# nanless/universal-speech-enhancement

Hardware: AMD Instinct MI355X
Metric: spectrogram-frames/sec through 30-step PC sampler, 24 kHz (higher is better)
Workload: dtype bf16; 1 GPU; configs[1]: NCSN++ Large score net, batch=8x4 s utterances per GPU, 30-step PC sampler (reverse_diffusion + langevin x1, snr 0.5, 60 NFE), bf16, hipGraph=on; global_batch=8, frames_per_utt=601, padded_frames_per_utt=640, n_freq=512, N=30, nfe=60, parallelism=utterance-sharded x1

## Files before the change

universal_speech_enhancement_amd/csrc/use_conv_sk.hip:

```cpp
#include "use_kernels.h"
#include <type_traits>
#include "use_device.h"

namespace use {

namespace {

template <typename T> struct SkMma;
template <> struct SkMma<__bf16> {
    DEVI static f32x16 mma(const uint4 a, const uint4 b, f32x16 c) {
        return __builtin_amdgcn_mfma_f32_32x32x16_bf16(__builtin_bit_cast(bf16x8, a), __builtin_bit_cast(bf16x8, b), c, 0, 0, 0);
    }
};
template <> struct SkMma<_Float16> {
    DEVI static f32x16 mma(const uint4 a, const uint4 b, f32x16 c) {
        return __builtin_amdgcn_mfma_f32_32x32x16_f16(__builtin_bit_cast(f16x8, a), __builtin_bit_cast(f16x8, b), c, 0, 0, 0);
    }
};
template <> struct SkMma<float> {
    DEVI static f32x16 mma(const uint4 a, const uint4 b, f32x16 c) {
        const float4 fa = __builtin_bit_cast(float4, a), fb = __builtin_bit_cast(float4, b);
        c = __builtin_amdgcn_mfma_f32_32x32x2f32(fa.x, fb.x, c, 0, 0, 0);
        c = __builtin_amdgcn_mfma_f32_32x32x2f32(fa.y, fb.y, c, 0, 0, 0);
        c = __builtin_amdgcn_mfma_f32_32x32x2f32(fa.z, fb.z, c, 0, 0, 0);
        c = __builtin_amdgcn_mfma_f32_32x32x2f32(fa.w, fb.w, c, 0, 0, 0);
        return c;
    }
};

constexpr int SK_HPMAX = 128;
constexpr int SK_MT = 64;

template <typename TIN, typename TOUT, int NJ, int CP>
__global__ __launch_bounds__(512) void conv_sk_kernel(ConvArgs p, int TH, int TW) {
    constexpr int ES = (int)sizeof(TIN);
    constexpr int VEC = 16 / ES;
    constexpr int NP = ES;
    constexpr int MI = SK_MT / 32, MT = SK_MT, NT = 32 * NJ;
    constexpr int ROWB = CP * ES + 16;
    constexpr int UMAX = (9 * (CP / 32) + 7) / 8;
    constexpr int NPC = SK_HPMAX * (CP * ES / 16) / 512;
    constexpr int NTP = NT + 8;
    constexpr int HALO_BYTES = SK_HPMAX * ROWB, RED_BYTES = 4 * MT * NTP * 4;
    constexpr int SMEM = HALO_BYTES > RED_BYTES ? HALO_BYTES : RED_BYTES;
    constexpr bool ACC = ES == 4;
    static_assert(NPC >= 1 && SK_HPMAX * (CP * ES / 16) % 512 == 0, "halo staging");
    __shared__ __attribute__((aligned(16))) char smem[SMEM];
    __shared__ float2 coef_s[1024];
    __shared__ float2 st_red[8][NT];

    const int tid = threadIdx.x, lane = tid & 63, wave = tid >> 6;
    const int b = blockIdx.z, n0 = blockIdx.y * NT;
    const int pad = p.ntaps == 9 ? 1 : 0;
    const int tiles_x = (p.W + TW - 1) / TW;
    const int ty0 = (blockIdx.x / tiles_x) * TH, tx0 = (blockIdx.x % tiles_x) * TW;
    const int HW_ = TW + 2 * pad, HP = HW_ * (TH + 2 * pad);
    const int Ctot = p.C0 + p.C1, XCtot = p.XC0 + p.XC1;
    const bool has_gn = p.coef || p.gn_st0;

    f32x16 acc[MI][NJ];
#pragma unroll
    for (int i = 0; i < MI; ++i)
#pragma unroll
        for (int j = 0; j < NJ; ++j)
#pragma unroll
            for (int r = 0; r < 16; ++r) acc[i][j][r] = 0.f;

    int a_off[MI];
#pragma unroll
    for (int i = 0; i < MI; ++i) {
        int m = i * 32 + (lane & 31);
        if (m >= TH * TW) m = 0;
        const int ty = m / TW;
        a_off[i] = (ty * HW_ + (m - ty * TW)) * ROWB + (lane >> 5) * 16;
    }

    bool first = true;
    for (int si = 0; si < 4; ++si) {
        const bool seg1 = si >= 2;
        const TIN* src = (const TIN*)(si == 0 ? p.src0 : si == 1 ? p.src1 : si == 2 ? p.x0 : p.x1);
        const int Cs = si == 0 ? p.C0 : si == 1 ? p.C1 : si == 2 ? p.XC0 : p.XC1;
        const int cg0 = si == 1 ? p.C0 : si == 3 ? p.XC0 : 0;
        const char* wbase = seg1 ? (const char*)p.w2 : (const char*)p.w;
        const int wld = seg1 ? XCtot : Ctot, wtaps = seg1 ? 1 : p.ntaps;
        const bool use_coef = has_gn && !seg1, use_act = p.act && !seg1;
        const char* wslab = seg1 ? (const char*)p.w2b : (const char*)p.wb;
        constexpr int SCK = ES == 4 ? 16 : 32;
        const int nslabs = wld / SCK;
        for (int c_loc = 0; c_loc < Cs; c_loc += CP) {
            const int pc = Cs - c_loc < CP ? Cs - c_loc : CP;
            const int cpu_ = pc >> 5;
            const int nunits = wtaps * cpu_;
            const int c_glob = cg0 + c_loc;
            const int d_tap = 8 / cpu_, d_chunk = 8 - d_tap * cpu_;
            const int tap0 = wave / cpu_, chunk0 = wave - tap0 * cpu_;
            uint4 bw[UMAX][NJ][NP];
            {
                int tap = tap0, chunk = chunk0;
#pragma unroll
                for (int i = 0; i < UMAX; ++i) {
                    if (wave + 8 * i < nunits) {
#pragma unroll
                        for (int j = 0; j < NJ; ++j) {
                            int row = n0 + j * 32 + (lane & 31);
#ifdef USE_HIP_ABLATE
                            if (p.dbg & 1) row = n0 + j * 32 + (lane & 1);
#endif
                            if (wslab) {
#pragma unroll
                                for (int q = 0; q < NP; ++q) {
                                    const int cgl = c_glob + chunk * 32 + (2 * q + (lane >> 5)) * VEC;
                                    const int slab = cgl / SCK, piece = (cgl % SCK) / VEC;
                                    bw[i][j][q] = *reinterpret_cast<const uint4*>(
                                        wslab + (((size_t)tap * nslabs + slab) * p.cout_pad + row) * 64 + ((piece ^ ((row >> 2) & 3)) << 4));
                                }
                            } else {
                                const char* wp = wbase + (((size_t)row * wtaps + tap) * wld + c_glob + chunk * 32) * ES + (lane >> 5) * 16;
#pragma unroll
                                for (int q = 0; q < NP; ++q) bw[i][j][q] = *reinterpret_cast<const uint4*>(wp + q * 32);
                            }
                        }
                    }
                    tap += d_tap; chunk += d_chunk;
                    if (chunk >= cpu_) { chunk -= cpu_; ++tap; }
                }
            }
            if (first) {
                if (has_gn) gn_fill_table(coef_s, p, b, Ctot, tid, 512);
                first = false;
            }
            __syncthreads();
            const int ppp = pc * ES / 16;
            const int npieces = HP * ppp;
            const int d_pix = 512 / ppp, d_part = 512 - d_pix * ppp;
            const int d_hy = d_pix / HW_, d_hx = d_pix - d_hy * HW_;
            uint4 raw[NPC];
            int loff[NPC];
            {
                int pix = tid / ppp, part = tid - pix * ppp;
                int hy = pix / HW_, hx = pix - hy * HW_;
#pragma unroll
                for (int k = 0; k < NPC; ++k) {
                    raw[k] = make_uint4(0, 0, 0, 0);
                    loff[k] = 0;
                    if (tid + k * 512 < npieces) {
                        const int gy = ty0 + hy - pad, gx = tx0 + hx - pad;
                        const bool inb = gy >= 0 && gy < p.H && gx >= 0 && gx < p.W;
                        loff[k] = (pix * ROWB + part * 16) | (inb ? 0x40000000 : 0) | 0x80000000;
                        if (inb) raw[k] = *reinterpret_cast<const uint4*>(src + ((size_t)(b * p.H + gy) * p.W + gx) * Cs + c_loc + part * VEC);
                    }
                    part += d_part; pix += d_pix; hx += d_hx; hy += d_hy;
                    if (part >= ppp) { part -= ppp; ++pix; ++hx; }
                    if (hx >= HW_) { hx -= HW_; ++hy; }
                }
            }
            {
                int part = tid % ppp;
#pragma unroll
                for (int k = 0; k < NPC; ++k) {
                    if (loff[k] < 0) {
                        uint4 o = raw[k];
#ifdef USE_HIP_ABLATE
                        if (p.dbg & 2) { *reinterpret_cast<uint4*>(smem + (loff[k] & 0x3fffffff)) = o; continue; }
#endif
                        if ((loff[k] & 0x40000000) && (use_coef || use_act)) {
                            float v[VEC];
                            Vec16<TIN>::load(reinterpret_cast<const TIN*>(&o), v);
                            if (use_coef) {
                                const float2* cf = coef_s + c_glob + part * VEC;
#pragma unroll
                                for (int e = 0; e < VEC; ++e) { const float2 ab = cf[e]; v[e] = fmaf(v[e], ab.x, ab.y); }
                            }
                            if (use_act) {
#pragma unroll
                                for (int e = 0; e < VEC; ++e) v[e] = silu_f<ACC>(v[e]);
                            }
                            o = Vec16<TIN>::pack(v);
                        }
                        *reinterpret_cast<uint4*>(smem + (loff[k] & 0x3fffffff)) = o;
                    }
                    part += d_part;
                    if (part >= ppp) part -= ppp;
                }
            }
            __syncthreads();
            {
                int tap = tap0, chunk = chunk0;
#pragma unroll
                for (int i = 0; i < UMAX; ++i) {
#ifdef USE_HIP_ABLATE
                    if (p.dbg & 4) { if (wave + 8 * i < nunits) { _Pragma("unroll") for (int j = 0; j < NJ; ++j) _Pragma("unroll") for (int q = 0; q < NP; ++q) acc[0][j][q] += __builtin_bit_cast(float, bw[i][j][q].x); } continue; }
#endif
                    if (wave + 8 * i < nunits) {
                        const int dy = seg1 ? pad : (pad ? (tap * 11) >> 5 : 0);
                        const int dx = seg1 ? pad : (pad ? tap - dy * 3 : 0);
                        const char* ha = smem + (dy * HW_ + dx) * ROWB + chunk * 32 * ES;
#pragma unroll
                        for (int q = 0; q < NP; ++q) {
                            uint4 af[MI];
#pragma unroll
                            for (int m = 0; m < MI; ++m) af[m] = *reinterpret_cast<const uint4*>(ha + a_off[m] + q * 32);
#pragma unroll
                            for (int m = 0; m < MI; ++m)
#pragma unroll
                                for (int j = 0; j < NJ; ++j) acc[m][j] = SkMma<TIN>::mma(af[m], bw[i][j][q], acc[m][j]);
                        }
                    }
                    tap += d_tap; chunk += d_chunk;
                    if (chunk >= cpu_) { chunk -= cpu_; ++tap; }
                }
            }
        }
    }

    float* const red = reinterpret_cast<float*>(smem);
    float* const mine = red + (wave & 3) * (MT * NTP);
    __syncthreads();
#define SK_FOR_ACC(BODY)                                                                                   \
    _Pragma("unroll") for (int m = 0; m < MI; ++m) _Pragma("unroll") for (int j = 0; j < NJ; ++j)          \
    _Pragma("unroll") for (int r = 0; r < 16; ++r) {                                                       \
        const int row = m * 32 + (r & 3) + 8 * (r >> 2) + 4 * (lane >> 5), col = j * 32 + (lane & 31);     \
        BODY;                                                                                              \
    }
    if (wave >= 4) { SK_FOR_ACC(mine[row * NTP + col] = acc[m][j][r]) }
    __syncthreads();
    if (wave < 4) { SK_FOR_ACC(mine[row * NTP + col] += acc[m][j][r]) }
    __syncthreads();
#undef SK_FOR_ACC

    constexpr int CH = 16 / (int)sizeof(TOUT);
    constexpr int CPR = NT / CH;
    constexpr int ITEMS = MT * CPR;
    static_assert(512 % CPR == 0 && (CPR == 4 || CPR == 8 || CPR == 16), "epilogue chunking");
    TOUT* out = (TOUT*)p.out;
    const TOUT* res = (const TOUT*)p.res;
    const int ch = tid % CPR;
    const int co0 = n0 + ch * CH;
    float addv[CH], st_s[CH], st_q[CH];
    const int nvalid = p.Cout - co0;
#pragma unroll
    for (int c = 0; c < CH; ++c) {
        float add = 0.f;
        if (c < nvalid) {
            if (p.bias) add += p.bias[co0 + c];
            if (p.temb) add += p.temb[(size_t)b * p.temb_bstride + co0 + c];
        }
        addv[c] = add; st_s[c] = 0.f; st_q[c] = 0.f;
    }
#pragma unroll
    for (int it0 = 0; it0 < ITEMS; it0 += 512) {
        const int it = it0 + tid;
        const int row = it / CPR;
        if (it < ITEMS && row < TH * TW && nvalid > 0) {
            const int ty = row / TW, gy = ty0 + ty, gx = tx0 + row - ty * TW;
            if (gy < p.H && gx < p.W) {
                float v[CH];
#pragma unroll
                for (int c = 0; c < CH; ++c) v[c] = addv[c];
#pragma unroll
                for (int w = 0; w < 4; ++w)
#pragma unroll
                    for (int c4 = 0; c4 < CH / 4; ++c4) {
                        const float4 t4 = *reinterpret_cast<const float4*>(red + w * (MT * NTP) + row * NTP + ch * CH + c4 * 4);
                        v[c4 * 4] += t4.x; v[c4 * 4 + 1] += t4.y; v[c4 * 4 + 2] += t4.z; v[c4 * 4 + 3] += t4.w;
                    }
                const size_t pix = (size_t)(b * p.H + gy) * p.W + gx;
                if (res) {
                    float rv[CH];
                    if (nvalid >= CH) Vec16<TOUT>::load(res + pix * p.Cout + co0, rv);
                    else {
#pragma unroll
                        for (int c = 0; c < CH; ++c) rv[c] = c < nvalid ? to_f(res[pix * p.Cout + co0 + c]) : 0.f;
                    }
#pragma unroll
                    for (int c = 0; c < CH; ++c) v[c] += rv[c];
                }
#pragma unroll
                for (int c = 0; c < CH; ++c) v[c] *= p.out_scale;
                if (p.pyr && nvalid >= CH) {
                    const float4 pq = *reinterpret_cast<const float4*>(p.pyr + pix * 4);
#pragma unroll
                    for (int c = 0; c < CH; ++c) {
                        const float4 wq = *reinterpret_cast<const float4*>(p.w4 + (size_t)(co0 + c) * 4);
                        v[c] += p.b4[co0 + c] + wq.x * pq.x + wq.y * pq.y + wq.z * pq.z + wq.w * pq.w;
                    }
                }
                const uint4 packed = Vec16<TOUT>::pack(v);
                if (nvalid >= CH) *reinterpret_cast<uint4*>(out + pix * p.Cout + co0) = packed;
                else {
#pragma unroll
                    for (int c = 0; c < CH; ++c) if (c < nvalid) out[pix * p.Cout + co0 + c] = reinterpret_cast<const TOUT*>(&packed)[c];
                }
                float vr[CH];
                Vec16<TOUT>::load(reinterpret_cast<const TOUT*>(&packed), vr);
#pragma unroll
                for (int c = 0; c < CH; ++c) { st_s[c] += vr[c]; st_q[c] += vr[c] * vr[c]; }
            }
        }
    }
    if (p.stats) {
        constexpr int NWV = ITEMS / 64 < 8 ? ITEMS / 64 : 8;
#pragma unroll
        for (int c = 0; c < CH; ++c) { st_s[c] = reduce_lanes_stride<CPR>(st_s[c]); st_q[c] = reduce_lanes_stride<CPR>(st_q[c]); }
        if (lane < CPR && wave < NWV) {
#pragma unroll
            for (int c = 0; c < CH; ++c) st_red[wave][ch * CH + c] = make_float2(st_s[c], st_q[c]);
        }
        __syncthreads();
        if (tid < NT) {
            float ss = 0.f, qq = 0.f;
#pragma unroll
            for (int w = 0; w < NWV; ++w) { const float2 t = st_red[w][tid]; ss += t.x; qq += t.y; }
            if (n0 + tid < p.Cout) gn_accumulate(p.stats + ((size_t)b * p.Cout + n0 + tid) * 2, ss, qq);
        }
    }
}

long g_sk_max_px = 16L * 20L;

void sk_tile(int H, int W, int pad, int* th, int* tw) {
    long best = -1; int bh = 1, bw = 1;
    for (int w = 1; w <= W && w <= SK_MT; ++w) {
        int hmax = SK_MT / w; if (hmax > H) hmax = H;
        const int ny = (H + hmax - 1) / hmax;
        const int h = (H + ny - 1) / ny;
        const int halo = (h + 2 * pad) * (w + 2 * pad);
        if (halo > SK_HPMAX) continue;
        const long tiles = (long)ny * ((W + w - 1) / w);
        const long key = tiles * 1024 + halo;
        if (best < 0 || key < best) { best = key; bh = h; bw = w; }
    }
    *th = bh; *tw = bw;
}

template <typename T, typename TO, int NJ, int CP>
void sk_launch(const ConvArgs& a, int th, int tw, hipStream_t s) {
    const int tiles = ((a.H + th - 1) / th) * ((a.W + tw - 1) / tw);
    hipLaunchKernelGGL((conv_sk_kernel<T, TO, NJ, CP>), dim3(tiles, (a.Cout + 32 * NJ - 1) / (32 * NJ), a.B), dim3(512), 0, s, a, th, tw);
}

}

void conv_sk_set_max_px(long n) { g_sk_max_px = n; }

bool conv_sk_eligible(const ConvArgs& a) {
    const int Ctot = a.C0 + a.C1, XC = a.XC0 + a.XC1;
    const bool full = a.in_dtype == a.out_dtype && a.Cout % 32 == 0 && a.Cout >= 32;
    const bool head = a.out_dtype == DT_F32 && a.Cout <= 8 && a.cout_pad >= 32 && !a.pyr && !a.stats;
    const long max_px = (a.in_dtype == DT_F32 && g_sk_max_px > 0) ? std::max(g_sk_max_px, 4096L) : g_sk_max_px;
    return (long)a.H * a.W <= max_px && (a.ntaps == 9 || a.ntaps == 1) && a.w && (full || head) &&
           Ctot % 32 == 0 && a.C0 % 32 == 0 && XC % 32 == 0 && a.XC0 % 32 == 0 && (XC == 0 || a.w2) && Ctot >= 32 && Ctot <= 1024;
}

void launch_conv_sk(const ConvArgs& a, hipStream_t s) {
    int th, tw;
    sk_tile(a.H, a.W, a.ntaps == 9 ? 1 : 0, &th, &tw);
    const long tiles = (long)((a.H + th - 1) / th) * ((a.W + tw - 1) / tw) * a.B;
    const bool wide = a.Cout % 64 == 0 && tiles * (a.Cout / 32) > 512;
    if (a.in_dtype != a.out_dtype) {
        if (a.in_dtype == DT_BF16) sk_launch<__bf16, float, 1, 256>(a, th, tw, s); else sk_launch<_Float16, float, 1, 256>(a, th, tw, s);
        return;
    }
    if (a.in_dtype == DT_BF16)     { wide ? sk_launch<__bf16, __bf16, 2, 128>(a, th, tw, s) : sk_launch<__bf16, __bf16, 1, 256>(a, th, tw, s); }
    else if (a.in_dtype == DT_F16) { wide ? sk_launch<_Float16, _Float16, 2, 128>(a, th, tw, s) : sk_launch<_Float16, _Float16, 1, 256>(a, th, tw, s); }
    else                           { wide ? sk_launch<float, float, 2, 64>(a, th, tw, s) : sk_launch<float, float, 1, 128>(a, th, tw, s); }
}

}
```

universal_speech_enhancement_amd/csrc/use_engine.cpp:

```cpp
#include "../../include/use_hip.h"
#include "use_kernels.h"

#include <hip/hip_runtime.h>

#include <algorithm>
#include <cmath>
#include <cstdarg>
#include <cstdio>
#include <cstdlib>
#include <cstring>
#include <map>
#include <mutex>
#include <string>
#include <unordered_map>
#include <vector>

using namespace use;

static thread_local std::string g_err;
static int fail(int code, const char* fmt, ...) {
    char buf[1024];
    va_list ap; va_start(ap, fmt); vsnprintf(buf, sizeof buf, fmt, ap); va_end(ap);
    g_err = buf;
    return code;
// ... 810 lines not shown
}

static int ensure_sde_scratch(use_handle* h) {
    if (!h) return fail(USE_E_INVALID, "null handle");
    HIPCHK(hipSetDevice(h->device));
    if (!h->sde_buf) {
        const size_t bytes = 512 + (size_t)use_handle::SDE_MAX_B * use_handle::SDE_BLOCKS * 2 * 4;
        HIPCHK(hipMalloc((void**)&h->sde_buf, bytes));
        HIPCHK(hipMemset(h->sde_buf, 0, bytes));
        h->sde_rng = (unsigned long long*)h->sde_buf; h->sde_step = (float*)(h->sde_buf + 256);
        h->sde_partial = (float*)(h->sde_buf + 512);
    }
    return USE_OK;
}

static int ensure_cap_stream(use_handle* h) {
    if (!h->cap_stream) HIPCHK(hipStreamCreateWithFlags(&h->cap_stream, hipStreamNonBlocking));
    return USE_OK;
}

extern "C" {

int use_get_stat(use_handle* h, const char* name, long long* value) {
    if (!h || !name || !value) return fail(USE_E_INVALID, "null argument");
    if (!strcmp(name, "graph_captures")) { *value = h->n_graph_captures; return USE_OK; }
    if (!strcmp(name, "plans_built")) { *value = h->n_plans_built; return USE_OK; }
    if (!strcmp(name, "plan_cache_hits")) { *value = h->n_plan_cache_hits; return USE_OK; }
    if (!strcmp(name, "plans_parked")) { *value = (long long)h->plan_cache.size(); return USE_OK; }
    if (!strcmp(name, "ode_steps")) { *value = h->ode_steps; return USE_OK; }
    if (!strcmp(name, "ode_rejected")) { *value = h->ode_rejected; return USE_OK; }
    if (!strcmp(name, "ode_nfev_max")) { *value = h->ode_nfev_max; return USE_OK; }
    if (!strcmp(name, "plan_stale")) { *value = h->B && h->opt_gen_at_plan != g_opt_gen ? 1 : 0; return USE_OK; }
    return fail(USE_E_INVALID, "unknown statistic '%s'", name);
}

int use_set_option(const char* name, long long value) {
    if (!name) return fail(USE_E_INVALID, "option name is null");
    ++g_opt_gen;
    if (!strcmp(name, "attn_fused")) { g_attn_fused = (int)value; return USE_OK; }
    if (!strcmp(name, "plan_cache")) { g_plan_cache = (int)std::max(0LL, std::min(16LL, value)); return USE_OK; }
    if (!strcmp(name, "subbatch_min_items")) { g_subbatch_min_items = (int)std::max(1LL, value); return USE_OK; }
    if (!strcmp(name, "subbatch")) { g_subbatch = (int)value; return USE_OK; }
    if (!strcmp(name, "stagger_level")) { g_stagger_level = (int)value; return USE_OK; }
    if (!strcmp(name, "stats_part")) { g_stats_part = (int)value; return USE_OK; }
    if (!strcmp(name, "gn_inline")) { g_gn_inline = (long)value; return USE_OK; }
    if (!strcmp(name, "conv_v4_min_blocks")) { conv_v4_set_min_blocks((long)value); return USE_OK; }
    if (!strcmp(name, "conv_v5")) { conv_v5_set((int)value); return USE_OK; }
    if (!strcmp(name, "fir_strip")) { fir_set_strip((int)value); return USE_OK; }
    if (!strcmp(name, "pyr_ws")) { pyr_conv_set_ws((int)value); return USE_OK; }
    if (!strcmp(name, "wgrad_mfma16")) { wgrad_set_mfma16((int)value); return USE_OK; }
    if (!strcmp(name, "wgrad_blocks")) { wgrad_set_blocks((int)value); return USE_OK; }
    if (!strcmp(name, "conv_in_wgs")) { if (value < 1 || value > 4096) return fail(USE_E_INVALID, "conv_in_wgs: 1 ... 4096"); g_conv_in_wgs = (int)value; return USE_OK; }
    if (!strcmp(name, "conv_sk_max_px")) { conv_sk_set_max_px((long)value); return USE_OK; }
    return fail(USE_E_INVALID, "unknown option '%s'", name);
}
const char* use_last_error(void) { return g_err.c_str(); }
const char* use_version(void) { return "use_hip 0.1 (gfx950)"; }

int use_create(const use_config* cfg, int device, use_handle** out) {
    if (!cfg || !out) return fail(USE_E_INVALID, "null argument");
    if (cfg->n_levels < 1 || cfg->n_levels > 8 || cfg->nf % 32 != 0 || cfg->nf < 32 || cfg->num_res_blocks < 1)
        return fail(USE_E_INVALID, "unsupported architecture (nf must be a multiple of 32, 1..8 levels)");
    for (int i = 0; i < cfg->n_levels; ++i)
        if (cfg->ch_mult[i] < 1 || cfg->nf * cfg->ch_mult[i] > 512) return fail(USE_E_INVALID, "unsupported architecture (1 <= nf * ch_mult <= 512)");
    if (cfg->n_freq % (1 << (cfg->n_levels - 1)) != 0)
        return fail(USE_E_INVALID, "n_freq=%d is not divisible by 2^(levels-1)", cfg->n_freq);
    if (cfg->precision != USE_PREC_FP32 && cfg->precision != USE_PREC_BF16 && cfg->precision != USE_PREC_FP16) return fail(USE_E_INVALID, "bad precision");
    if (cfg->input_channels != 0 && cfg->input_channels != 2 && cfg->input_channels != 4 && cfg->input_channels != 6)
        return fail(USE_E_INVALID, "input_channels must be 4 (x and y), 6 (x, y and a second conditioning) or 2 (y alone), got %d", cfg->input_channels);
    use_handle* h = new use_handle();
    h->cfg = *cfg; h->device = device;
    h->act_dtype = cfg->precision == USE_PREC_BF16 ? DT_BF16 : cfg->precision == USE_PREC_FP16 ? DT_F16 : DT_F32;
    int rc = build_arch(h);
    if (rc) { delete h; return rc; }
    *out = h;
    return USE_OK;
}

int use_destroy(use_handle* h) {
    if (!h) return USE_OK;
    (void)hipSetDevice(h->device);
    (void)hipDeviceSynchronize();
    drop_graphs(h); plan_cache_clear(h);
    if (h->ode_run) (void)use_ode_destroy(h->ode_run);
    if (h->cap_stream) (void)hipStreamDestroy(h->cap_stream);
    for (int i = 0; i < MAX_SUB; ++i) {
        if (h->aux_stream[i]) (void)hipStreamDestroy(h->aux_stream[i]);
        if (h->ev_stagger[i]) { (void)hipEventDestroy(h->ev_stagger[i]); (void)hipEventDestroy(h->ev_join[i]); }
    }
    if (h->ev_fork) (void)hipEventDestroy(h->ev_fork);
    if (h->blob) (void)hipFree(h->blob);
    if (h->arena.base) (void)hipFree(h->arena.base);
    if (h->persist) (void)hipFree(h->persist);
    if (h->temb_table) (void)hipFree(h->temb_table);
    if (h->silu_table) (void)hipFree(h->silu_table);
    if (h->ts_dev) (void)hipFree(h->ts_dev);
    if (h->noise_copy) (void)hipFree(h->noise_copy);
    if (h->sde_buf) (void)hipFree(h->sde_buf);
    delete h;
    return USE_OK;
}

int use_num_expected_weights(use_handle* h) { return h ? (int)h->expected.size() : USE_E_INVALID; }
int use_expected_weight(use_handle* h, int index, const char** name, int64_t* shape4, int* ndim) {
    if (!h || index < 0 || index >= (int)h->expected.size()) return fail(USE_E_INVALID, "bad index");
    const Expected& e = h->expected[index];
// ... 1319 lines not shown
```

universal_speech_enhancement_amd/csrc/use_kernels.h:

```cpp
#pragma once
#include <hip/hip_runtime.h>
#include <stdint.h>
#include <atomic>
#include <thread>

namespace use {

constexpr int USE_MAX_DEVICES = 64;
struct LdsAttrOnce {
    std::atomic<int> st[USE_MAX_DEVICES] = {};
    template <typename F> void once(F&& f) {
        int d = 0;
        if (hipGetDevice(&d) != hipSuccess || d < 0 || d >= USE_MAX_DEVICES) { f(); return; }
        if (st[d].load(std::memory_order_acquire) == 2) return;
        int expected = 0;
        if (st[d].compare_exchange_strong(expected, 1, std::memory_order_acq_rel)) { f(); st[d].store(2, std::memory_order_release); }
        else while (st[d].load(std::memory_order_acquire) != 2) std::this_thread::yield();
    }
    template <typename K> void operator()(K kern, int bytes) {
        once([&] { (void)hipFuncSetAttribute(reinterpret_cast<const void*>(kern), hipFuncAttributeMaxDynamicSharedMemorySize, bytes); });
    }
};


enum DType { DT_F32 = 0, DT_BF16 = 1, DT_F16 = 2 };
inline size_t dtype_size(int dt) { return dt == DT_F32 ? 4 : 2; }

constexpr int CONV_IN_SPLIT_K = 112;
constexpr int TILE_H = 8;
constexpr int TILE_W = 16;

inline int tiles_per_image(int H, int W) { return ((H + TILE_H - 1) / TILE_H) * ((W + TILE_W - 1) / TILE_W); }
extern int g_conv_in_wgs;
inline int conv_in_split_tpw(int H, int W) { const int nt = tiles_per_image(H, W); return (nt + g_conv_in_wgs - 1) / g_conv_in_wgs; }
inline int conv_in_split_wgs(int H, int W) { const int nt = tiles_per_image(H, W), tpw = conv_in_split_tpw(H, W); return (nt + tpw - 1) / tpw; }
inline int conv_v2_tiles(int H, int W) { return ((H + 15) / 16) * ((W + 15) / 16); }

struct ConvArgs {
    const void* src0; const void* src1; int C0; int C1; int in_dtype;
    const float* coef;
    const long long* gn_st0; const long long* gn_st1;
    const float* gn_gamma; const float* gn_beta; int gn_groups; float gn_inv_n; float gn_eps;
    int act;
    const void* w;
    const void* wb;
    int cout_pad;
    const void* x0; const void* x1; int XC0; int XC1; const void* w2;
    const void* w2b;
    const float* bias;
    const float* temb;
    int temb_bstride;
    const void* res;
    float out_scale;
    const float* pyr;
    const float* w4;
    const float* b4;
    void* out; int out_dtype;
    long long* stats_part;
    long long* stats;
    int B, H, W, Cout, ntaps;
    int dbg;
    unsigned long long* trace;
};
void launch_conv(const ConvArgs& a, hipStream_t s);
int conv_stats_parts(const ConvArgs& a);
bool conv_v2_eligible(const ConvArgs& a);
void launch_conv_v2(const ConvArgs& a, hipStream_t s);
inline int conv_v4_chunk(int dtype) { return dtype == DT_F32 ? 16 : 32; }
inline int conv_v4_tiles(int H, int W) { return ((H + 15) / 16) * ((W + 31) / 32); }
bool conv_sk_eligible(const ConvArgs& a);
void conv_sk_set_max_px(long n);
void launch_conv_sk(const ConvArgs& a, hipStream_t s);
void launch_conv_generic(const ConvArgs& a, hipStream_t s);
void pyr_conv_set_ws(int n);
bool conv_v4_eligible(const ConvArgs& a);
const char* conv_v4_unrunnable(const ConvArgs& a);
void conv_v4_set_min_blocks(long n);
void launch_conv_v4(const ConvArgs& a, hipStream_t s);
const char* conv_v5_unrunnable(const ConvArgs& a);
void conv_v5_set(int on);
bool conv_v5_enabled(const ConvArgs& a);
void launch_conv_v5(const ConvArgs& a, hipStream_t s);
void launch_gn_finalize(const long long* st0, int C0, const long long* st1, int C1, const float* gamma, const float* beta,
                        int groups, int hw, float eps, float* coef, int B, hipStream_t s, const long long* pt0 = nullptr, int nt0 = 0,
                        const long long* pt1 = nullptr, int nt1 = 0);

void launch_fir_up2(const void* src, int dtype, const float* coef, int act, void* out_act, void* out_raw, int B,
                    int H, int W, int C, hipStream_t s);
void fir_set_strip(int on);
void launch_fir_down2(const void* src, int dtype, const float* coef, int act, void* out_act, void* out_raw, int B,
                      int H, int W, int C, hipStream_t s);

void launch_spec_map(const float2* in, float2* out, long rows, int Tin, int Tin_stride, int Tout, float pre, float power,
                     float post, hipStream_t s);

void launch_twiddle_table(float2* tw, int N, hipStream_t s);
void launch_stft_fwd(const float* wav, const float* win, const float2* tw, float2* Y, int B, int L, int N, int hop, int T,
                     int Tpad, float factor, float expo, hipStream_t s);
void launch_istft_back(const float2* X, const float* win, const float2* tw, float* wav, int B, int L, int N, int hop, int Tpad,
                       float factor, float expo, hipStream_t s);

void launch_pack_input(const float2* x, const float2* y, const float2* y2, float* x4, long npix, hipStream_t s);
void launch_combine_add(void* h, int dtype, const float* pyr, const float* w8, const float* b8, long long* stats, int B, long pix_per_b,
                        int C, hipStream_t s);

void launch_temb_mlp(const float* t, int t_stride, const float* gfp_w, const float* w1, const float* b1,
                     const float* w2, const float* b2, float* out_silu, int B, int nf, hipStream_t s);
void launch_temb_dense(const float* silu_temb, const float* W, const float* bias, float* out, int B, int rows,
                       int dim, hipStream_t s);

void launch_attention(const void* q, const void* k, const void* v, void* out, int dtype, int B, int N, int C,
                      hipStream_t s);

struct AttnArgs {
    const void* x; void* out; int N;
    const long long* gn_st; const float* gn_gamma; const float* gn_beta; int gn_groups; float gn_eps;
    const void *wq, *wk, *wv, *wo; const float *bq, *bk, *bv, *bo;
    long long* stats;
};
bool attn_fused_eligible(int dtype, int N, int C);
void launch_attn_fused(const AttnArgs& a, int dtype, int B, hipStream_t s);

void launch_softmax_rows(void* x, int dtype, long rows, int cols, hipStream_t s);
void launch_transpose_nc(const void* in, void* out, int dtype, int B, int N, int C, hipStream_t s);
// ... 72 lines not shown
```

Baseline: 3604 spectrogram-frames/s.

## Software-pipeline halo and weight loads in split-K conv kernel

Adds a prefetching variant of the split-K conv kernel, on by default. It issues the next channel pass's halo loads into registers before the current pass's MFMA work, and loads the next weights right after the barrier. Bias, temb and residual values for the epilogue are also fetched early. Full __syncthreads are replaced with lgkmcnt-only waits plus s_barrier, to hide global-load latency behind compute. The cost is extra register pressure (raw halo, weights and epilogue buffers all live together), which may reduce occupancy.

```diff
diff --git a/universal_speech_enhancement_amd/csrc/use_conv_sk.hip b/universal_speech_enhancement_amd/csrc/use_conv_sk.hip
--- a/universal_speech_enhancement_amd/csrc/use_conv_sk.hip
+++ b/universal_speech_enhancement_amd/csrc/use_conv_sk.hip
@@ -31,7 +31,9 @@
 constexpr int SK_HPMAX = 128;
 constexpr int SK_MT = 64;
 
-template <typename TIN, typename TOUT, int NJ, int CP>
+#define SK_LDS_BARRIER() asm volatile("s_waitcnt lgkmcnt(0)\n\ts_barrier" ::: "memory")
+
+template <typename TIN, typename TOUT, int NJ, int CP, bool PF>
 __global__ __launch_bounds__(512) void conv_sk_kernel(ConvArgs p, int TH, int TW) {
     constexpr int ES = (int)sizeof(TIN);
     constexpr int VEC = 16 / ES;
@@ -57,6 +59,35 @@
     const int HW_ = TW + 2 * pad, HP = HW_ * (TH + 2 * pad);
     const int Ctot = p.C0 + p.C1, XCtot = p.XC0 + p.XC1;
     const bool has_gn = p.coef || p.gn_st0;
+    constexpr int CH = 16 / (int)sizeof(TOUT);
+    constexpr int CPR = NT / CH;
+    constexpr int ITEMS = MT * CPR;
+    constexpr int NIT = (ITEMS + 511) / 512;
+    static_assert(512 % CPR == 0 && (CPR == 4 || CPR == 8 || CPR == 16), "epilogue chunking");
+    TOUT* out = (TOUT*)p.out;
+    const TOUT* res = (const TOUT*)p.res;
+    const int ch = tid % CPR;
+    const int co0 = n0 + ch * CH;
+    const int nvalid = p.Cout - co0;
+    float e_bias[CH], e_temb[CH];
+    uint4 e_res[NIT];
+
+#ifdef USE_HIP_TRACE_BUILD
+    __shared__ unsigned long long trace_s[2][128];
+    const bool tracing = p.trace != nullptr && (int)(blockIdx.x + gridDim.x * blockIdx.z) == p.dbg && blockIdx.y == 0 && lane == 0 && (wave & 3) == 0;
+    int trace_n = 0, trace_pass = 0;
+    unsigned long long* const trace_lds = trace_s[wave >> 2];
+#define SK_STAMP(ID)                                                                                   \
+    if (tracing && trace_n < 64) {                                                                     \
+        trace_lds[2 * trace_n] = (unsigned long long)(ID);                                             \
+        trace_lds[2 * trace_n + 1] = __builtin_readcyclecounter(); ++trace_n;                          \
+    }
+#define SK_TRACE_NEXT_PASS ++trace_pass;
+#else
+#define SK_STAMP(ID)
+#define SK_TRACE_NEXT_PASS
+#endif
+    SK_STAMP(1)
 
     f32x16 acc[MI][NJ];
 #pragma unroll
@@ -75,147 +106,339 @@
         a_off[i] = (ty * HW_ + (m - ty * TW)) * ROWB + (lane >> 5) * 16;
     }
 
-    bool first = true;
-    for (int si = 0; si < 4; ++si) {
-        const bool seg1 = si >= 2;
-        const TIN* src = (const TIN*)(si == 0 ? p.src0 : si == 1 ? p.src1 : si == 2 ? p.x0 : p.x1);
-        const int Cs = si == 0 ? p.C0 : si == 1 ? p.C1 : si == 2 ? p.XC0 : p.XC1;
-        const int cg0 = si == 1 ? p.C0 : si == 3 ? p.XC0 : 0;
-        const char* wbase = seg1 ? (const char*)p.w2 : (const char*)p.w;
-        const int wld = seg1 ? XCtot : Ctot, wtaps = seg1 ? 1 : p.ntaps;
-        const bool use_coef = has_gn && !seg1, use_act = p.act && !seg1;
-        const char* wslab = seg1 ? (const char*)p.w2b : (const char*)p.wb;
+    if constexpr (PF) {
         constexpr int SCK = ES == 4 ? 16 : 32;
-        const int nslabs = wld / SCK;
-        for (int c_loc = 0; c_loc < Cs; c_loc += CP) {
-            const int pc = Cs - c_loc < CP ? Cs - c_loc : CP;
-            const int cpu_ = pc >> 5;
-            const int nunits = wtaps * cpu_;
-            const int c_glob = cg0 + c_loc;
-            const int d_tap = 8 / cpu_, d_chunk = 8 - d_tap * cpu_;
-            const int tap0 = wave / cpu_, chunk0 = wave - tap0 * cpu_;
-            uint4 bw[UMAX][NJ][NP];
-            {
-                int tap = tap0, chunk = chunk0;
-#pragma unroll
-                for (int i = 0; i < UMAX; ++i) {
-                    if (wave + 8 * i < nunits) {
-#pragma unroll
-                        for (int j = 0; j < NJ; ++j) {
-                            int row = n0 + j * 32 + (lane & 31);
-#ifdef USE_HIP_ABLATE
-                            if (p.dbg & 1) row = n0 + j * 32 + (lane & 1);
-#endif
-                            if (wslab) {
-#pragma unroll
-                                for (int q = 0; q < NP; ++q) {
-                                    const int cgl = c_glob + chunk * 32 + (2 * q + (lane >> 5)) * VEC;
-                                    const int slab = cgl / SCK, piece = (cgl % SCK) / VEC;
-                                    bw[i][j][q] = *reinterpret_cast<const uint4*>(
-                                        wslab + (((size_t)tap * nslabs + slab) * p.cout_pad + row) * 64 + ((piece ^ ((row >> 2) & 3)) << 4));
-                                }
-                            } else {
-                                const char* wp = wbase + (((size_t)row * wtaps + tap) * wld + c_glob + chunk * 32) * ES + (lane >> 5) * 16;
-#pragma unroll
-                                for (int q = 0; q < NP; ++q) bw[i][j][q] = *reinterpret_cast<const uint4*>(wp + q * 32);
+        struct SkPass {
+            const TIN* src; const char* wbase; const char* wslab;
+            int Cs, c_loc, c_glob, pc, cpu_, nunits, wld, nslabs, wtaps, d_tap, d_chunk, tap0, chunk0;
+            bool seg1;
+        };
+        typedef uint4 bw_t[UMAX][NJ][NP];
+        typedef uint4 raw_t[NPC];
+        typedef int loff_t[NPC];
+        int nx_si = 0, nx_c = 0;
+        auto next_pass = [&](SkPass& q) -> bool {
+            for (; nx_si < 4; ++nx_si, nx_c = 0) {
+                const int si = nx_si;
+                const int Cs = si == 0 ? p.C0 : si == 1 ? p.C1 : si == 2 ? p.XC0 : p.XC1;
+                if (nx_c >= Cs) continue;
+                q.seg1 = si >= 2;
+                q.src = (const TIN*)(si == 0 ? p.src0 : si == 1 ? p.src1 : si == 2 ? p.x0 : p.x1);
+                q.Cs = Cs; q.c_loc = nx_c;
+                q.c_glob = (si == 1 ? p.C0 : si == 3 ? p.XC0 : 0) + nx_c;
+                q.wbase = q.seg1 ? (const char*)p.w2 : (const char*)p.w;
+                q.wslab = q.seg1 ? (const char*)p.w2b : (const char*)p.wb;
+                q.wld = q.seg1 ? XCtot : Ctot; q.wtaps = q.seg1 ? 1 : p.ntaps;
+                q.nslabs = q.wld / SCK;
+                q.pc = Cs - nx_c < CP ? Cs - nx_c : CP;
+                q.cpu_ = q.pc >> 5;
+                q.nunits = q.wtaps * q.cpu_;
+                q.d_tap = 8 / q.cpu_; q.d_chunk = 8 - q.d_tap * q.cpu_;
+                q.tap0 = wave / q.cpu_; q.chunk0 = wave - q.tap0 * q.cpu_;
+                nx_c += CP;
+                return true;
+            }
+            return false;
+        };
+        auto load_w = [&](const SkPass& q, bw_t& bw) {
+            int tap = q.tap0, chunk = q.chunk0;
+#pragma unroll
+            for (int i = 0; i < UMAX; ++i) {
+                if (wave + 8 * i < q.nunits) {
+#pragma unroll
+                    for (int j = 0; j < NJ; ++j) {
+                        const int row = n0 + j * 32 + (lane & 31);
+                        if (q.wslab) {
+#pragma unroll
+                            for (int u = 0; u < NP; ++u) {
+                                const int cgl = q.c_glob + chunk * 32 + (2 * u + (lane >> 5)) * VEC;
+                                const int slab = cgl / SCK, piece = (cgl % SCK) / VEC;
+                                bw[i][j][u] = *reinterpret_cast<const uint4*>(
+                                    q.wslab + (((size_t)tap * q.nslabs + slab) * p.cout_pad + row) * 64 + ((piece ^ ((row >> 2) & 3)) << 4));
                             }
+                        } else {
+                            const char* wp = q.wbase + (((size_t)row * q.wtaps + tap) * q.wld + q.c_glob + chunk * 32) * ES + (lane >> 5) * 16;
+#pragma unroll
+                            for (int u = 0; u < NP; ++u) bw[i][j][u] = *reinterpret_cast<const uint4*>(wp + u * 32);
                         }
                     }
-                    tap += d_tap; chunk += d_chunk;
-                    if (chunk >= cpu_) { chunk -= cpu_; ++tap; }
-                }
-            }
-            if (first) {
-                if (has_gn) gn_fill_table(coef_s, p, b, Ctot, tid, 512);
-                first = false;
-            }
-            __syncthreads();
-            const int ppp = pc * ES / 16;
+                }
+                tap += q.d_tap; chunk += q.d_chunk;
+                if (chunk >= q.cpu_) { chunk -= q.cpu_; ++tap; }
+            }
+        };
+        auto load_halo = [&](const SkPass& q, raw_t& raw, loff_t& loff) {
+            const int ppp = q.pc * ES / 16;
             const int npieces = HP * ppp;
             const int d_pix = 512 / ppp, d_part = 512 - d_pix * ppp;
             const int d_hy = d_pix / HW_, d_hx = d_pix - d_hy * HW_;
-            uint4 raw[NPC];
-            int loff[NPC];
-            {
-                int pix = tid / ppp, part = tid - pix * ppp;
-                int hy = pix / HW_, hx = pix - hy * HW_;
-#pragma unroll
-                for (int k = 0; k < NPC; ++k) {
-                    raw[k] = make_uint4(0, 0, 0, 0);
-                    loff[k] = 0;
-                    if (tid + k * 512 < npieces) {
-                        const int gy = ty0 + hy - pad, gx = tx0 + hx - pad;
-                        const bool inb = gy >= 0 && gy < p.H && gx >= 0 && gx < p.W;
-                        loff[k] = (pix * ROWB + part * 16) | (inb ? 0x40000000 : 0) | 0x80000000;
-                        if (inb) raw[k] = *reinterpret_cast<const uint4*>(src + ((size_t)(b * p.H + gy) * p.W + gx) * Cs + c_loc + part * VEC);
-                    }
-                    part += d_part; pix += d_pix; hx += d_hx; hy += d_hy;
-                    if (part >= ppp) { part -= ppp; ++pix; ++hx; }
-                    if (hx >= HW_) { hx -= HW_; ++hy; }
-                }
-            }
-            {
-                int part = tid % ppp;
-#pragma unroll
-                for (int k = 0; k < NPC; ++k) {
-                    if (loff[k] < 0) {
-                        uint4 o = raw[k];
+            int pix = tid / ppp, part = tid - pix * ppp;
+            int hy = pix / HW_, hx = pix - hy * HW_;
+#pragma unroll
+            for (int k = 0; k < NPC; ++k) {
+                raw[k] = make_uint4(0, 0, 0, 0);
+                loff[k] = 0;
+                if (tid + k * 512 < npieces) {
+                    const int gy = ty0 + hy - pad, gx = tx0 + hx - pad;
+                    const bool inb = gy >= 0 && gy < p.H && gx >= 0 && gx < p.W;
+                    loff[k] = (pix * ROWB + part * 16) | (inb ? 0x40000000 : 0) | 0x80000000;
+                    if (inb) raw[k] = *reinterpret_cast<const uint4*>(q.src + ((size_t)(b * p.H + gy) * p.W + gx) * q.Cs + q.c_loc + part * VEC);
+                }
+                part += d_part; pix += d_pix; hx += d_hx; hy += d_hy;
+                if (part >= ppp) { part -= ppp; ++pix; ++hx; }
+                if (hx >= HW_) { hx -= HW_; ++hy; }
+            }
+        };
+        auto transform = [&](const SkPass& q, const raw_t& raw, const loff_t& loff) {
+            const bool use_coef = has_gn && !q.seg1, use_act = p.act && !q.seg1;
+            const int ppp = q.pc * ES / 16;
+            const int d_pix = 512 / ppp, d_part = 512 - d_pix * ppp;
+            int part = tid % ppp;
+#pragma unroll
+            for (int k = 0; k < NPC; ++k) {
+                if (loff[k] < 0) {
+                    uint4 o = raw[k];
+                    if ((loff[k] & 0x40000000) && (use_coef || use_act)) {
+                        float v[VEC];
+                        Vec16<TIN>::load(reinterpret_cast<const TIN*>(&o), v);
+                        if (use_coef) {
+                            const float2* cf = coef_s + q.c_glob + part * VEC;
+#pragma unroll
+                            for (int e = 0; e < VEC; ++e) { const float2 ab = cf[e]; v[e] = fmaf(v[e], ab.x, ab.y); }
+                        }
+                        if (use_act) {
+#pragma unroll
+                            for (int e = 0; e < VEC; ++e) v[e] = silu_f<ACC>(v[e]);
+                        }
+                        o = Vec16<TIN>::pack(v);
+                    }
+                    *reinterpret_cast<uint4*>(smem + (loff[k] & 0x3fffffff)) = o;
+                }
+                part += d_part;
+                if (part >= ppp) part -= ppp;
+            }
+        };
+        auto mma = [&](const SkPass& q, const bw_t& bw) {
+            int tap = q.tap0, chunk = q.chunk0;
+#pragma unroll
+            for (int i = 0; i < UMAX; ++i) {
+                if (wave + 8 * i < q.nunits) {
+                    const int dy = q.seg1 ? pad : (pad ? (tap * 11) >> 5 : 0);
+                    const int dx = q.seg1 ? pad : (pad ? tap - dy * 3 : 0);
+                    const char* ha = smem + (dy * HW_ + dx) * ROWB + chunk * 32 * ES;
+#pragma unroll
+                    for (int u = 0; u < NP; ++u) {
+                        uint4 af[MI];
+#pragma unroll
+                        for (int m = 0; m < MI; ++m) af[m] = *reinterpret_cast<const uint4*>(ha + a_off[m] + u * 32);
+#pragma unroll
+                        for (int m = 0; m < MI; ++m)
+#pragma unroll
+                            for (int j = 0; j < NJ; ++j) acc[m][j] = SkMma<TIN>::mma(af[m], bw[i][j][u], acc[m][j]);
+                    }
+                }
+                tap += q.d_tap; chunk += q.d_chunk;
+                if (chunk >= q.cpu_) { chunk -= q.cpu_; ++tap; }
+            }
+        };
+        auto load_epi = [&]() {
+#pragma unroll
+            for (int c = 0; c < CH; ++c) {
+                e_bias[c] = 0.f; e_temb[c] = 0.f;
+                if (c < nvalid) {
+                    if (p.bias) e_bias[c] = p.bias[co0 + c];
+                    if (p.temb) e_temb[c] = p.temb[(size_t)b * p.temb_bstride + co0 + c];
+                }
+            }
+#pragma unroll
+            for (int i = 0; i < NIT; ++i) {
+                e_res[i] = make_uint4(0, 0, 0, 0);
+                const int it = i * 512 + tid;
+                const int row = it / CPR;
+                if (res && it < ITEMS && row < TH * TW && nvalid >= CH) {
+                    const int ty = row / TW, gy = ty0 + ty, gx = tx0 + row - ty * TW;
+                    if (gy < p.H && gx < p.W) e_res[i] = *reinterpret_cast<const uint4*>(res + ((size_t)(b * p.H + gy) * p.W + gx) * p.Cout + co0);
+                }
+            }
+        };
+        SkPass cur, nxt;
+        bw_t bw;
+        raw_t raw;
+        loff_t loff;
+        next_pass(cur);
+        load_w(cur, bw);
+        load_halo(cur, raw, loff);
+        __builtin_amdgcn_sched_barrier(0);
+        if (has_gn) gn_fill_table(coef_s, p, b, Ctot, tid, 512);
+        SK_LDS_BARRIER();
+        SK_STAMP(2)
+        for (;;) {
+            __builtin_amdgcn_s_waitcnt(0x0f70);
+            SK_STAMP(30 + trace_pass)
+            transform(cur, raw, loff);
+            const bool more = next_pass(nxt);
+            if (more) load_halo(nxt, raw, loff);
+            SK_STAMP(40 + trace_pass)
+            SK_LDS_BARRIER();
+            SK_STAMP(10 + trace_pass)
+            mma(cur, bw);
+            SK_STAMP(20 + trace_pass)
+            SK_TRACE_NEXT_PASS
+            if (!more) break;
+            SK_LDS_BARRIER();
+            load_w(nxt, bw);
+            cur = nxt;
+        }
+        load_epi();
+    } else {
+        bool first = true;
+        for (int si = 0; si < 4; ++si) {
+            const bool seg1 = si >= 2;
+            const TIN* src = (const TIN*)(si == 0 ? p.src0 : si == 1 ? p.src1 : si == 2 ? p.x0 : p.x1);
+            const int Cs = si == 0 ? p.C0 : si == 1 ? p.C1 : si == 2 ? p.XC0 : p.XC1;
+            const int cg0 = si == 1 ? p.C0 : si == 3 ? p.XC0 : 0;
+            const char* wbase = seg1 ? (const char*)p.w2 : (const char*)p.w;
+            const int wld = seg1 ? XCtot : Ctot, wtaps = seg1 ? 1 : p.ntaps;
+            const bool use_coef = has_gn && !seg1, use_act = p.act && !seg1;
+            const char* wslab = seg1 ? (const char*)p.w2b : (const char*)p.wb;
+            constexpr int SCK = ES == 4 ? 16 : 32;
+            const int nslabs = wld / SCK;
+            for (int c_loc = 0; c_loc < Cs; c_loc += CP) {
+                const int pc = Cs - c_loc < CP ? Cs - c_loc : CP;
+                const int cpu_ = pc >> 5;
+                const int nunits = wtaps * cpu_;
+                const int c_glob = cg0 + c_loc;
+                const int d_tap = 8 / cpu_, d_chunk = 8 - d_tap * cpu_;
+                const int tap0 = wave / cpu_, chunk0 = wave - tap0 * cpu_;
+                uint4 bw[UMAX][NJ][NP];
+                {
+                    int tap = tap0, chunk = chunk0;
+#pragma unroll
+                    for (int i = 0; i < UMAX; ++i) {
+                        if (wave + 8 * i < nunits) {
+#pragma unroll
+                            for (int j = 0; j < NJ; ++j) {
+                                int row = n0 + j * 32 + (lane & 31);
 #ifdef USE_HIP_ABLATE
-                        if (p.dbg & 2) { *reinterpret_cast<uint4*>(smem + (loff[k] & 0x3fffffff)) = o; continue; }
+                                if (p.dbg & 1) row = n0 + j * 32 + (lane & 1);
 #endif
-                        if ((loff[k] & 0x40000000) && (use_coef || use_act)) {
-                            float v[VEC];
-                            Vec16<TIN>::load(reinterpret_cast<const TIN*>(&o), v);
-                            if (use_coef) {
-                                const float2* cf = coef_s + c_glob + part * VEC;
-#pragma unroll
-                                for (int e = 0; e < VEC; ++e) { const float2 ab = cf[e]; v[e] = fmaf(v[e], ab.x, ab.y); }
+                                if (wslab) {
+#pragma unroll
+                                    for (int q = 0; q < NP; ++q) {
+                                        const int cgl = c_glob + chunk * 32 + (2 * q + (lane >> 5)) * VEC;
+                                        const int slab = cgl / SCK, piece = (cgl % SCK) / VEC;
+                                        bw[i][j][q] = *reinterpret_cast<const uint4*>(
+                                            wslab + (((size_t)tap * nslabs + slab) * p.cout_pad + row) * 64 + ((piece ^ ((row >> 2) & 3)) << 4));
+                                    }
+                                } else {
+                                    const char* wp = wbase + (((size_t)row * wtaps + tap) * wld + c_glob + chunk * 32) * ES + (lane >> 5) * 16;
+#pragma unroll
+                                    for (int q = 0; q < NP; ++q) bw[i][j][q] = *reinterpret_cast<const uint4*>(wp + q * 32);
+                                }
                             }
-                            if (use_act) {
-#pragma unroll
-                                for (int e = 0; e < VEC; ++e) v[e] = silu_f<ACC>(v[e]);
+                        }
+                        tap += d_tap; chunk += d_chunk;
+                        if (chunk >= cpu_) { chunk -= cpu_; ++tap; }
+                    }
+                }
+                if (first) {
+                    if (has_gn) gn_fill_table(coef_s, p, b, Ctot, tid, 512);
+                    first = false;
+                }
+                __syncthreads();
+                SK_STAMP(30 + trace_pass)
+                const int ppp = pc * ES / 16;
+                const int npieces = HP * ppp;
+                const int d_pix = 512 / ppp, d_part = 512 - d_pix * ppp;
+                const int d_hy = d_pix / HW_, d_hx = d_pix - d_hy * HW_;
+                uint4 raw[NPC];
+                int loff[NPC];
+                {
+                    int pix = tid / ppp, part = tid - pix * ppp;
+                    int hy = pix / HW_, hx = pix - hy * HW_;
+#pragma unroll
+                    for (int k = 0; k < NPC; ++k) {
+                        raw[k] = make_uint4(0, 0, 0, 0);
+                        loff[k] = 0;
+                        if (tid + k * 512 < npieces) {
+                            const int gy = ty0 + hy - pad, gx = tx0 + hx - pad;
+                            const bool inb = gy >= 0 && gy < p.H && gx >= 0 && gx < p.W;
+                            loff[k] = (pix * ROWB + part * 16) | (inb ? 0x40000000 : 0) | 0x80000000;
+                            if (inb) raw[k] = *reinterpret_cast<const uint4*>(src + ((size_t)(b * p.H + gy) * p.W + gx) * Cs + c_loc + part * VEC);
+                        }
+                        part += d_part; pix += d_pix; hx += d_hx; hy += d_hy;
+                        if (part >= ppp) { part -= ppp; ++pix; ++hx; }
+                        if (hx >= HW_) { hx -= HW_; ++hy; }
+                    }
+                }
+                {
+                    int part = tid % ppp;
+#pragma unroll
+                    for (int k = 0; k < NPC; ++k) {
+                        if (loff[k] < 0) {
+                            uint4 o = raw[k];
+#ifdef USE_HIP_ABLATE
+                            if (p.dbg & 2) { *reinterpret_cast<uint4*>(smem + (loff[k] & 0x3fffffff)) = o; continue; }
+#endif
+                            if ((loff[k] & 0x40000000) && (use_coef || use_act)) {
+                                float v[VEC];
+                                Vec16<TIN>::load(reinterpret_cast<const TIN*>(&o), v);
+                                if (use_coef) {
+                                    const float2* cf = coef_s + c_glob + part * VEC;
+#pragma unroll
+                                    for (int e = 0; e < VEC; ++e) { const float2 ab = cf[e]; v[e] = fmaf(v[e], ab.x, ab.y); }
+                                }
+                                if (use_act) {
+#pragma unroll
+                                    for (int e = 0; e < VEC; ++e) v[e] = silu_f<ACC>(v[e]);
+                                }
+                                o = Vec16<TIN>::pack(v);
                             }
-                            o = Vec16<TIN>::pack(v);
+                            *reinterpret_cast<uint4*>(smem + (loff[k] & 0x3fffffff)) = o;
                         }
-                        *reinterpret_cast<uint4*>(smem + (loff[k] & 0x3fffffff)) = o;
-                    }
-                    part += d_part;
-                    if (part >= ppp) part -= ppp;
-                }
-            }
-            __syncthreads();
-            {
-                int tap = tap0, chunk = chunk0;
-#pragma unroll
-                for (int i = 0; i < UMAX; ++i) {
+                        part += d_part;
+                        if (part >= ppp) part -= ppp;
+                    }
+                }
+                SK_STAMP(40 + trace_pass)
+                __syncthreads();
+                SK_STAMP(10 + trace_pass)
+                {
+                    int tap = tap0, chunk = chunk0;
+#pragma unroll
+                    for (int i = 0; i < UMAX; ++i) {
 #ifdef USE_HIP_ABLATE
-                    if (p.dbg & 4) { if (wave + 8 * i < nunits) { _Pragma("unroll") for (int j = 0; j < NJ; ++j) _Pragma("unroll") for (int q = 0; q < NP; ++q) acc[0][j][q] += __builtin_bit_cast(float, bw[i][j][q].x); } continue; }
+                        if (p.dbg & 4) { if (wave + 8 * i < nunits) { _Pragma("unroll") for (int j = 0; j < NJ; ++j) _Pragma("unroll") for (int q = 0; q < NP; ++q) acc[0][j][q] += __builtin_bit_cast(float, bw[i][j][q].x); } continue; }
 #endif
-                    if (wave + 8 * i < nunits) {
-                        const int dy = seg1 ? pad : (pad ? (tap * 11) >> 5 : 0);
-                        const int dx = seg1 ? pad : (pad ? tap - dy * 3 : 0);
-                        const char* ha = smem + (dy * HW_ + dx) * ROWB + chunk * 32 * ES;
-#pragma unroll
-                        for (int q = 0; q < NP; ++q) {
-                            uint4 af[MI];
-#pragma unroll
-                            for (int m = 0; m < MI; ++m) af[m] = *reinterpret_cast<const uint4*>(ha + a_off[m] + q * 32);
-#pragma unroll
-                            for (int m = 0; m < MI; ++m)
-#pragma unroll
-                                for (int j = 0; j < NJ; ++j) acc[m][j] = SkMma<TIN>::mma(af[m], bw[i][j][q], acc[m][j]);
+                        if (wave + 8 * i < nunits) {
+                            const int dy = seg1 ? pad : (pad ? (tap * 11) >> 5 : 0);
+                            const int dx = seg1 ? pad : (pad ? tap - dy * 3 : 0);
+                            const char* ha = smem + (dy * HW_ + dx) * ROWB + chunk * 32 * ES;
+#pragma unroll
+                            for (int q = 0; q < NP; ++q) {
+                                uint4 af[MI];
+#pragma unroll
+                                for (int m = 0; m < MI; ++m) af[m] = *reinterpret_cast<const uint4*>(ha + a_off[m] + q * 32);
+#pragma unroll
+                                for (int m = 0; m < MI; ++m)
+#pragma unroll
+                                    for (int j = 0; j < NJ; ++j) acc[m][j] = SkMma<TIN>::mma(af[m], bw[i][j][q], acc[m][j]);
+                            }
                         }
-                    }
-                    tap += d_tap; chunk += d_chunk;
-                    if (chunk >= cpu_) { chunk -= cpu_; ++tap; }
-                }
+                        tap += d_tap; chunk += d_chunk;
+                        if (chunk >= cpu_) { chunk -= cpu_; ++tap; }
+                    }
+                }
+                SK_STAMP(20 + trace_pass)
+                SK_TRACE_NEXT_PASS
             }
         }
     }
 
     float* const red = reinterpret_cast<float*>(smem);
     float* const mine = red + (wave & 3) * (MT * NTP);
-    __syncthreads();
+#define SK_BAR() { if constexpr (PF) SK_LDS_BARRIER(); else __syncthreads(); }
+    SK_BAR()
 #define SK_FOR_ACC(BODY)                                                                                   \
     _Pragma("unroll") for (int m = 0; m < MI; ++m) _Pragma("unroll") for (int j = 0; j < NJ; ++j)          \
     _Pragma("unroll") for (int r = 0; r < 16; ++r) {                                                       \
@@ -223,27 +446,24 @@
         BODY;                                                                                              \
     }
     if (wave >= 4) { SK_FOR_ACC(mine[row * NTP + col] = acc[m][j][r]) }
-    __syncthreads();
+    SK_BAR()
     if (wave < 4) { SK_FOR_ACC(mine[row * NTP + col] += acc[m][j][r]) }
-    __syncthreads();
+    SK_BAR()
 #undef SK_FOR_ACC
-
-    constexpr int CH = 16 / (int)sizeof(TOUT);
-    constexpr int CPR = NT / CH;
-    constexpr int ITEMS = MT * CPR;
-    static_assert(512 % CPR == 0 && (CPR == 4 || CPR == 8 || CPR == 16), "epilogue chunking");
-    TOUT* out = (TOUT*)p.out;
-    const TOUT* res = (const TOUT*)p.res;
-    const int ch = tid % CPR;
-    const int co0 = n0 + ch * CH;
+    SK_STAMP(5)
+
     float addv[CH], st_s[CH], st_q[CH];
-    const int nvalid = p.Cout - co0;
 #pragma unroll
     for (int c = 0; c < CH; ++c) {
         float add = 0.f;
         if (c < nvalid) {
-            if (p.bias) add += p.bias[co0 + c];
-            if (p.temb) add += p.temb[(size_t)b * p.temb_bstride + co0 + c];
+            if constexpr (PF) {
+                if (p.bias) add += e_bias[c];
+                if (p.temb) add += e_temb[c];
+            } else {
+                if (p.bias) add += p.bias[co0 + c];
+                if (p.temb) add += p.temb[(size_t)b * p.temb_bstride + co0 + c];
+            }
         }
         addv[c] = add; st_s[c] = 0.f; st_q[c] = 0.f;
     }
@@ -267,7 +487,10 @@
                 const size_t pix = (size_t)(b * p.H + gy) * p.W + gx;
                 if (res) {
                     float rv[CH];
-                    if (nvalid >= CH) Vec16<TOUT>::load(res + pix * p.Cout + co0, rv);
+                    if (nvalid >= CH) {
+                        if constexpr (PF) Vec16<TOUT>::load(reinterpret_cast<const TOUT*>(&e_res[it0 / 512]), rv);
+                        else Vec16<TOUT>::load(res + pix * p.Cout + co0, rv);
+                    }
                     else {
 #pragma unroll
                         for (int c = 0; c < CH; ++c) rv[c] = c < nvalid ? to_f(res[pix * p.Cout + co0 + c]) : 0.f;
@@ -298,6 +521,7 @@
             }
         }
     }
+    SK_STAMP(6)
     if (p.stats) {
         constexpr int NWV = ITEMS / 64 < 8 ? ITEMS / 64 : 8;
 #pragma unroll
@@ -306,7 +530,7 @@
 #pragma unroll
             for (int c = 0; c < CH; ++c) st_red[wave][ch * CH + c] = make_float2(st_s[c], st_q[c]);
         }
-        __syncthreads();
+        SK_BAR()
         if (tid < NT) {
             float ss = 0.f, qq = 0.f;
 #pragma unroll
@@ -314,8 +538,18 @@
             if (n0 + tid < p.Cout) gn_accumulate(p.stats + ((size_t)b * p.Cout + n0 + tid) * 2, ss, qq);
         }
     }
+#undef SK_BAR
+    SK_STAMP(7)
+#ifdef USE_HIP_TRACE_BUILD
+    if (tracing) {
+        for (int i = 0; i < 2 * trace_n; ++i) p.trace[(wave >> 2) * 256 + i] = trace_lds[i];
+    }
+#endif
+#undef SK_STAMP
+#undef SK_TRACE_NEXT_PASS
 }
 
+int g_sk_prefetch = 1;
 long g_sk_max_px = 16L * 20L;
 
 void sk_tile(int H, int W, int pad, int* th, int* tw) {
@@ -336,12 +570,15 @@
 template <typename T, typename TO, int NJ, int CP>
 void sk_launch(const ConvArgs& a, int th, int tw, hipStream_t s) {
     const int tiles = ((a.H + th - 1) / th) * ((a.W + tw - 1) / tw);
-    hipLaunchKernelGGL((conv_sk_kernel<T, TO, NJ, CP>), dim3(tiles, (a.Cout + 32 * NJ - 1) / (32 * NJ), a.B), dim3(512), 0, s, a, th, tw);
+    const dim3 grid(tiles, (a.Cout + 32 * NJ - 1) / (32 * NJ), a.B);
+    if (g_sk_prefetch) hipLaunchKernelGGL((conv_sk_kernel<T, TO, NJ, CP, true>), grid, dim3(512), 0, s, a, th, tw);
+    else hipLaunchKernelGGL((conv_sk_kernel<T, TO, NJ, CP, false>), grid, dim3(512), 0, s, a, th, tw);
 }
 
 }
 
 void conv_sk_set_max_px(long n) { g_sk_max_px = n; }
+void conv_sk_set_prefetch(int on) { g_sk_prefetch = on != 0; }
 
 bool conv_sk_eligible(const ConvArgs& a) {
     const int Ctot = a.C0 + a.C1, XC = a.XC0 + a.XC1;
diff --git a/universal_speech_enhancement_amd/csrc/use_engine.cpp b/universal_speech_enhancement_amd/csrc/use_engine.cpp
--- a/universal_speech_enhancement_amd/csrc/use_engine.cpp
+++ b/universal_speech_enhancement_amd/csrc/use_engine.cpp
@@ -886,6 +886,7 @@
     if (!strcmp(name, "wgrad_blocks")) { wgrad_set_blocks((int)value); return USE_OK; }
     if (!strcmp(name, "conv_in_wgs")) { if (value < 1 || value > 4096) return fail(USE_E_INVALID, "conv_in_wgs: 1 ... 4096"); g_conv_in_wgs = (int)value; return USE_OK; }
     if (!strcmp(name, "conv_sk_max_px")) { conv_sk_set_max_px((long)value); return USE_OK; }
+    if (!strcmp(name, "conv_sk_prefetch")) { conv_sk_set_prefetch((int)value); return USE_OK; }
     return fail(USE_E_INVALID, "unknown option '%s'", name);
 }
 const char* use_last_error(void) { return g_err.c_str(); }
diff --git a/universal_speech_enhancement_amd/csrc/use_kernels.h b/universal_speech_enhancement_amd/csrc/use_kernels.h
--- a/universal_speech_enhancement_amd/csrc/use_kernels.h
+++ b/universal_speech_enhancement_amd/csrc/use_kernels.h
@@ -70,6 +70,7 @@
 inline int conv_v4_tiles(int H, int W) { return ((H + 15) / 16) * ((W + 31) / 32); }
 bool conv_sk_eligible(const ConvArgs& a);
 void conv_sk_set_max_px(long n);
+void conv_sk_set_prefetch(int on);
 void launch_conv_sk(const ConvArgs& a, hipStream_t s);
 void launch_conv_generic(const ConvArgs& a, hipStream_t s);
 void pyr_conv_set_ws(int n);
```

Measured after the change: 3604 spectrogram-frames/s, median of 2. Within noise of the previous version (+0.0%).
